# NUSTM/FacialMMT

Hardware: AMD Instinct MI355X
Metric: utterances/sec T+A+V forward+bwd, 160-frame face seq, 1/2/4/8 GPU (higher is better)
Workload: dtype bf16; 1 GPU; configs[1]: T+A+V, RoBERTa-large (random init), 160-frame face seq (uint8 112x112 crops, fused pil-bicubic x2 + normalise), batch 4 utterances/GPU, bf16, fwd+bwd+clip+AdamW every step; global_batch=4, parallelism=dp1, hip_graphs=whole step: 2 graphs (fwd+bwd | clip+optimizer), text_encoder_concurrent_with_swin=True, swin_forward_pipelined_across_steps=False, text_encoder_parameters=bf16 with fp32 master weights in the optimizer

## Files before the change

### facialmmt_amd/_lib.py

```python
from __future__ import annotations

import ctypes as C
import os

_HERE = os.path.dirname(os.path.abspath(__file__))
LIB_PATH = os.path.join(_HERE, "libfmmt_hip.so")

F32, BF16 = 0, 1
GENERIC = 0x100
EPI_NONE, EPI_GELU, EPI_GELU_BWD, EPI_GELU_DG, EPI_MUL_AUX = 0, 1, 2, 3, 4
SAVE_DG = 0x200
BATCH_MAJOR = 0x400
RESIZE_PIL, RESIZE_CV2 = 0, 1

_p, _i, _f, _sz, _u64 = C.c_void_p, C.c_int, C.c_float, C.c_size_t, C.c_uint64

SIGNATURES = {
    "fmmt_version": (_i, []),
    "fmmt_linear_fwd": (_i, [_i, _i, _i, _i, _p, _i, _p, _i, _p, _p, _i, _p, _i, _p, _i, _p, _i, _p, _i, _p]),
    "fmmt_linear_splitk_workspace": (_sz, [_i, _i, _i]),
    "fmmt_linear_fwd_splitk": (_i, [_i, _i, _i, _i, _p, _i, _p, _i, _p, _p, _i, _p, _sz, _p]),
    "fmmt_linear_wgrad_workspace": (_sz, [_i, _i, _i, _i]),
    "fmmt_linear_wgrad": (_i, [_i, _i, _i, _i, _p, _i, _p, _i, _p, _p, _p, _i, _i, _p, _sz, _p]),
    "fmmt_linear_wgrad_partials": (_i, [_i, _i, _i, _i, _p, _i, _p, _i, _i, _p, _i, _i, _p, _sz, _p]),
# ... 86 lines not shown
DIGEST_WORDS = 6

EVAL_SHARD_SIGNATURES = {
    "fmmt_eval_accumulate_rows": (_i, [_i, _i, _i, _p, _i, _p, _p, _p, _p, _p, _p, _p, _p, _p, C.c_int64, _p]),
    "fmmt_eval_merge": (_i, [_i, _i, C.c_int64, C.c_int64, _p, _p, _p, _p, _p, _p, _p]),
}

JITTER_SIGNATURES = {
    "fmmt_jitter_table_check": (_i, [_p, _i]),
    "fmmt_patch_embed_u8_jitter": (_i, [_i, _i, _i, _i, _p, _p, _p, _p, _p, _p, _p]),
    "fmmt_patch_embed_u8_jitter_ln_fwd": (_i, [_i, _i, _i, _i, _p, _p, _p, _p, _p, _p, _p, _p, _p, _f, _p, _p, _p, _p, _p, _p]),
}
JITTER_WORDS, JITTER_BANDS = 8, 56
JITTER_BRIGHTNESS, JITTER_CONTRAST, JITTER_SATURATION, JITTER_HUE, JITTER_NONE = 0, 1, 2, 3, 4

AUG_SIGNATURES = {
    "fmmt_aug_table_check": (_i, [_p, _i]),
    "fmmt_aug_workspace_bytes": (C.c_size_t, [_i]),
    "fmmt_patch_embed_u8_aug": (_i, [_i, _i, _i, _i, _p, _p, _p, _p, _p, _p, C.c_size_t, _p, _p]),
    "fmmt_patch_embed_u8_aug_ln_fwd": (_i, [_i, _i, _i, _i, _p, _p, _p, _p, _p, _p, C.c_size_t, _p, _p, _p, _p, _f, _p, _p, _p, _p, _p, _p]),
}
AUG_WORDS, AUG_FLAG_GRAY, AUG_MAX_RADIUS, AUG_HALO = 20, 1, 1, 6

FMMT_EINVAL, FMMT_EALIGN, FMMT_EWORKSPACE = -1, -2, -3
_ERR = {-1: "FMMT_EINVAL (bad shape / unsupported size)", -2: "FMMT_EALIGN (pointer or leading dimension not 16-byte aligned)",
        -3: "FMMT_EWORKSPACE (workspace too small)"}

_lib = None


class FmmtError(RuntimeError):
    pass


def load():
    global _lib
    if _lib is not None:
        return _lib
    if not os.path.exists(LIB_PATH):
        raise FmmtError(f"{LIB_PATH} is missing: build it with `python -m facialmmt_amd.build` "
                        f"(or __graft_entry__.build()); there is no CPU / PyTorch fallback for the hot path")
    lib = C.CDLL(LIB_PATH)
    for name, (res, args) in list(SIGNATURES.items()) + list(POOL_HEAD_SIGNATURES.items()) + list(RAGGED_SIGNATURES.items()) + list(EVAL_COLLECT_SIGNATURES.items()) + list(POOL_HEAD_ROWS_SIGNATURES.items()) + list(GUARD_SIGNATURES.items()) + list(DIGEST_SIGNATURES.items()) + list(EVAL_SHARD_SIGNATURES.items()) + list(JITTER_SIGNATURES.items()) + list(AUG_SIGNATURES.items()):
        fn = getattr(lib, name)
        fn.restype = res
        fn.argtypes = args
    _lib = lib
    return lib


def check(rc: int, what: str):
    if rc != 0:
        msg = _ERR.get(rc, f"hipError_t {rc}")
        raise FmmtError(f"{what} failed: {msg}")


def dtype_code(t) -> int:
    import torch
    if t == torch.float32:
        return F32
    if t == torch.bfloat16:
        return BF16
    raise FmmtError(f"unsupported activation dtype {t}: the HIP path computes in float32 (parity) or bfloat16 (throughput)")
```

### facialmmt_amd/build.py

```python
from __future__ import annotations

import glob
import os
import subprocess
import sys
from concurrent.futures import ThreadPoolExecutor

HERE = os.path.dirname(os.path.abspath(__file__))
CSRC = os.path.join(HERE, "csrc")
OUT = os.path.join(HERE, "libfmmt_hip.so")
SOURCES = ["gemm.hip", "layernorm.hip", "attn.hip", "wattn_mfma.hip", "wattn_bwd_ref.hip", "wblock.hip", "wblock_ref.hip", "mha_mfma.hip", "misc.hip", "preproc.hip", "mlp_fused.hip", "mlp_ref.hip", "patch_ln.hip", "lin_lnbwd.hip", "plm_fused.hip", "frame_filter.hip", "eval.hip", "pool_head.hip", "ragged.hip", "guard.hip", "digest.hip", "eval_shard.hip", "color_jitter.hip", "aff_augment.hip"]
FLAGS = ["--offload-arch=gfx950", "-O3", "-std=c++17", "-fPIC", "-ffp-contract=fast"]


def _stale(target, deps):
    if not os.path.exists(target):
        return True
    t = os.path.getmtime(target)
    return any(os.path.getmtime(d) > t for d in deps)


def build(force: bool = False, verbose: bool = True, tag: str = "") -> str:
    hipcc = os.environ.get("HIPCC", "/opt/rocm/bin/hipcc")
    tag = tag or os.environ.get("FMMT_BUILD_TAG", "")
    csrc = os.environ.get("FMMT_CSRC_DIR", CSRC) if tag else CSRC
    headers = sorted(glob.glob(os.path.join(csrc, "*.h"))) + [os.path.join(csrc, "..", "..", "include", h) for h in ("fmmt.h", "fmmt_pool_head.h", "fmmt_ragged.h", "fmmt_eval_collect.h", "fmmt_pool_head_rows.h", "fmmt_guard.h", "fmmt_digest.h", "fmmt_eval_shard.h", "fmmt_jitter.h", "fmmt_aug.h")]
    objdir = os.path.join(HERE, "build_" + tag if tag else "build")
    out = os.path.join(HERE, f"libfmmt_hip_{tag}.so") if tag else OUT
    os.makedirs(objdir, exist_ok=True)
    jobs = []
    for s in SOURCES:
        src = os.path.join(csrc, s)
        obj = os.path.join(objdir, s.replace(".hip", ".o"))
        if force or _stale(obj, [src] + headers):
            jobs.append((src, obj))

    def cc(job):
        src, obj = job
        cmd = [hipcc] + FLAGS + os.environ.get("FMMT_CFLAGS", "").split() + ["-c", src, "-o", obj]
        if verbose:
            print(" ".join(cmd), flush=True)
        subprocess.run(cmd, check=True)

    with ThreadPoolExecutor(max_workers=4) as ex:
        list(ex.map(cc, jobs))
    objs = [os.path.join(objdir, s.replace(".hip", ".o")) for s in SOURCES]
    if force or jobs or _stale(out, objs):
        cmd = [hipcc, "--offload-arch=gfx950", "-shared", "-fPIC", "-o", out] + objs
        if verbose:
# ... 8 lines not shown
```

### facialmmt_amd/csrc/gemm.hip

```cpp
#include "gemm_common.h"
#include "gemm_ph.h"
#include "gemm_ph3.h"
#include <stdlib.h>
#include <type_traits>

namespace {

template <typename T> struct Mma;
template <> struct Mma<bf16> {
    static constexpr int KM = 32;
    static constexpr int KP = 8;
    using frag = bf16x8;
    static __device__ __forceinline__ f32x4 mma(frag a, frag b, f32x4 c) {
        return __builtin_amdgcn_mfma_f32_16x16x32_bf16(a, b, c, 0, 0, 0);
    }
    static __device__ __forceinline__ frag load(const bf16* p) { return *reinterpret_cast<const bf16x8*>(p); }
};
template <> struct Mma<float> {
    static constexpr int KM = 4;
    static constexpr int KP = 1;
    using frag = float;
    static __device__ __forceinline__ f32x4 mma(frag a, frag b, f32x4 c) {
        return __builtin_amdgcn_mfma_f32_16x16x4f32(a, b, c, 0, 0, 0);
    }
    static __device__ __forceinline__ frag load(const float* p) { return *p; }
};

__device__ __forceinline__ int xcd_remap(int bid, int nwg) {
    const int q = nwg >> 3, r = nwg & 7, xcd = bid & 7;
    return (xcd < r ? xcd * (q + 1) : r * (q + 1) + (xcd - r) * q) + (bid >> 3);
}

template <int BM, int NBUF> struct NtWaves { static constexpr int value = (BM == 128) ? (NBUF == 1 ? 3 : 2) : 4; };
template <typename T, int BM, int BN, int BK, int NBUF, bool GLDS, bool SEG = false>
__global__ __launch_bounds__(256) __attribute__((amdgpu_waves_per_eu(NtWaves<BM, NBUF>::value)))
void linear_nt_kernel(LinArgs p) {
    constexpr int VEC = Vec<T>::N;
    static_assert(!SEG || GLDS, "segmented weights: direct-to-LDS kernels only");
    constexpr int PITCH = GLDS ? BK : BK + VEC;
    constexpr int KM = Mma<T>::KM, KP = Mma<T>::KP;
    constexpr int WM = BM / 2, WN = BN / 2, MT = WM / 16, NT = WN / 16;
    constexpr int KV = BK / VEC;
    constexpr int W_VECS = BN * KV, X_VECS = BM * KV;
    constexpr int WV = (W_VECS + 255) / 256, XV = (X_VECS + 255) / 256;
    constexpr int CW = 4 * NT;

    extern __shared__ __attribute__((aligned(16))) char smem[];
    T* Ws = reinterpret_cast<T*>(smem);
    T* Xs = Ws + NBUF * BN * PITCH;

    const int tid = threadIdx.x, lane = tid & 63, wave = tid >> 6;
    const int wm = wave >> 1, wn = wave & 1;
    const int li = lane & 15, lg = lane >> 4;

    const T* __restrict__ xg = reinterpret_cast<const T*>(p.x);
    const T* __restrict__ wg = reinterpret_cast<const T*>(p.w);
    const float* bias_seg = nullptr;
    if constexpr (SEG) {
        if (p.wseg_mode == 1) {
            const int s_ = ((xcd_remap(blockIdx.x, gridDim.x) % p.tiles_n) * BN) / p.wseg;
            wg = reinterpret_cast<const T*>(s_ == 0 ? p.w : (s_ == 1 ? p.w1 : p.w2)) - (ptrdiff_t)s_ * p.wseg * p.ldw;
            const float* bs_ = s_ == 0 ? p.bias : (s_ == 1 ? p.bias1 : p.bias2);
            bias_seg = bs_ ? bs_ - (ptrdiff_t)s_ * p.wseg : nullptr;
        }
    }

    const int kbeg = p.ksplit ? blockIdx.y * p.ksplit : 0;
    const int kend = p.ksplit ? min(p.K, kbeg + p.ksplit) : p.K;
    const int nk = (kend - kbeg + BK - 1) / BK;

    struct Stage { Vec<T> w[WV], x[XV]; };
    Stage R0;

    auto gload = [&](Stage& R, int k0, int m0, int n0) {
#pragma unroll
        for (int i = 0; i < WV; ++i) {
            const int v = tid + i * 256;
            if (v < W_VECS) {
                const int row = v / KV, kc = (v % KV) * VEC;
                const int n = min(n0 + row, p.N - 1);
                R.w[i] = (k0 + kc < kend) ? ldvec<T>(wg + (size_t)n * p.ldw + k0 + kc) : zerovec<T>();
            }
        }
#pragma unroll
        for (int i = 0; i < XV; ++i) {
            const int v = tid + i * 256;
            if (v < X_VECS) {
                const int row = v / KV, kc = (v % KV) * VEC;
                const int m = min(m0 + row, p.M - 1);
                R.x[i] = (k0 + kc < kend) ? ldvec<T>(xg + (size_t)m * p.ldx + k0 + kc) : zerovec<T>();
            }
        }
// ... 44 lines not shown
#pragma unroll
            for (int a = 0; a < MT; ++a)
#pragma unroll
                for (int b = 0; b < NT; ++b) acc[a][b] = Mma<T>::mma(wf[b], xf[a], acc[a][b]);
        }
    };

    auto epilogue = [&](int m0, int n0) {
        if constexpr (SEG) {
            if (bias_seg) {
#pragma unroll
                for (int b = 0; b < NT; ++b) {
                    const f32x4 bb = *reinterpret_cast<const f32x4*>(bias_seg + n0 + wn * WN + chan_of<CW>(b, lg, 0));
#pragma unroll
                    for (int a = 0; a < MT; ++a) acc[a][b] += bb;
                }
            }
            nt_epilogue<T, MT, NT, true>(p, acc, m0 + wm * WM, n0 + wn * WN, li, lg);
        } else {
            nt_epilogue<T, MT, NT>(p, acc, m0 + wm * WM, n0 + wn * WN, li, lg);
        }
    };

    const int logical = xcd_remap(blockIdx.x, gridDim.x);
    const int m0 = (logical / p.tiles_n) * BM, n0 = (logical % p.tiles_n) * BN;
#pragma unroll
    for (int a = 0; a < MT; ++a)
#pragma unroll
        for (int b = 0; b < NT; ++b) acc[a][b] = f32x4{0.f, 0.f, 0.f, 0.f};
    if constexpr (GLDS) {
        static_assert(BK == 64 && (NBUF == 2 || NBUF == 4) && sizeof(T) == 2, "direct-to-LDS path: bf16, BK = 64, two or four buffers");
        typedef __attribute__((address_space(1))) const void gptr_t;
        typedef __attribute__((address_space(3))) void lptr_t;
        auto issue = [&](int buf, int k0) {
            const int r8 = lane >> 3, c = lane & 7;
            const T* wk = wg;
            int kw = k0;
            if constexpr (SEG) {
                if (p.wseg_mode == 2) {
                    const int s_ = k0 / p.wseg;
                    wk = reinterpret_cast<const T*>(s_ == 0 ? p.w : (s_ == 1 ? p.w1 : p.w2));
                    kw = k0 - s_ * p.wseg;
                }
            }
#pragma unroll
            for (int i = 0; i < BN / 32; ++i) {
                const int grp = i * 4 + wave, row = grp * 8 + r8;
// ... 31 lines not shown
            const int cur = kt & 1;
            if (kt + 1 < nk) issue(cur ^ 1, kbeg + (kt + 1) * BK);
            compute(cur);
            __syncthreads();
        }
        epilogue(m0, n0);
        return;
    }
    gload(R0, kbeg, m0, n0);
    lstore(R0, 0);
    __syncthreads();
    if constexpr (NBUF == 1) {
        compute(0);
    } else {
        for (int kt = 0; kt < nk; ++kt) {
            const int cur = kt & 1;
            if (kt + 1 < nk) gload(R0, kbeg + (kt + 1) * BK, m0, n0);
            compute(cur);
            if (kt + 1 < nk) lstore(R0, cur ^ 1);
            __syncthreads();
        }
    }
    epilogue(m0, n0);
}

__global__ __launch_bounds__(512) void linear_nt_deep_kernel(LinArgs p) {
    using T = bf16;
    constexpr int BM = 256, BN = 128, BK = 64, PITCH = 64, MT = 4, NT = 4, CW = 16;
    constexpr int STAGE = (BM + BN) * PITCH;
    extern __shared__ __attribute__((aligned(16))) char smem[];
    T* S = reinterpret_cast<T*>(smem);

    const int tid = threadIdx.x, lane = tid & 63, wave = tid >> 6;
    const int wm = wave >> 1, wn = wave & 1;
    const int li = lane & 15, lg = lane >> 4;
    const int logical = xcd_remap(blockIdx.x, gridDim.x);
    const int m0 = (logical / p.tiles_n) * BM, n0 = (logical % p.tiles_n) * BN;
    const T* __restrict__ xg = reinterpret_cast<const T*>(p.x);
    const T* __restrict__ wg = reinterpret_cast<const T*>(p.w);
    const int nk = p.K / BK;

    typedef __attribute__((address_space(1))) const void gptr_t;
    typedef __attribute__((address_space(3))) void lptr_t;
    const int r8 = lane >> 3, c = lane & 7;
    auto issue = [&](int buf, int k0) {
        T* base = S + buf * STAGE;
// ... 677 lines not shown
    if (a.rowscale && a.rows_per_scale <= 0) return 0;
    if ((unsigned long long)a.M * a.ldx >= (1ull << 31) || (unsigned long long)a.N * a.ldw >= (1ull << 31) || (unsigned long long)a.M * a.ldy >= (1ull << 31) ||
        (a.res && (unsigned long long)a.M * a.ldres >= (1ull << 31)))
        return 0;
    if (a.N % 256) {
        if (gelu_pre || a.K > 512) return 0;
        const long long t384 = (long long)((a.M + 383) / 384) * (a.N / 128), r384 = (t384 + 255) / 256;
        if (t384 < 256 || t384 * 100 < r384 * 256 * 85) return 0;
        *epi3 = mul_aux ? 6 : has_op ? 5 : 2;
        return 4;
    }
    const long long t256 = (long long)((a.M + 255) / 256) * (a.N / 256), t192 = (long long)((a.M + 191) / 192) * (a.N / 256);
    const long long r256 = (t256 + 255) / 256, r192 = (t192 + 255) / 256;
    const long long min_tiles = a.M < 16384 ? 150 : 256;
    const bool ok256 = t256 >= min_tiles && (a.M < 16384 || t256 * 100 >= r256 * 256 * 85);
    const bool ok192 = t192 >= min_tiles && (a.M < 16384 || t192 * 100 >= r192 * 256 * 85);
    *epi3 = gelu_pre ? 3 : mul_aux ? 6 : has_op ? 5 : 2;
    if (gelu_pre || has_op || mul_aux) return ok192 ? 3 : 0;
    const long long c256 = r256 * 256 * 100, c192 = r192 * 192 * 103;
    if (ok192 && (!ok256 || c192 < c256)) return 3;
    return ok256 ? 1 : 0;
}

template <typename T>
int dispatch_nt(const LinArgs& a, hipStream_t st) {
    const bool n96 = (a.N % 96 == 0) && (a.N % 128 != 0);
    if (a.M <= 4096 && (a.N < 16384 || a.M < 256)) {
        if constexpr (sizeof(T) == 2) {
            constexpr int SMALL_TILES = 256;
            constexpr int SMALL_R4K = 2048;
            const int tiles = ((a.M + 63) / 64) * ((a.N + 127) / 128);
            if (tiles < SMALL_TILES && a.N % 64 == 0 && a.K % 64 == 0 && a.K >= 128 && !a.ksplit && a.ldx % 8 == 0 && a.ldw % 8 == 0) {
                if (a.K >= SMALL_R4K) return launch_nt<T, 32, 64, 64, 4, true>(a, st);
                return launch_nt<T, 32, 64, 64, 2, true>(a, st);
            }
        }
        return n96 ? dispatch_nt_bk<T, 64, 96>(a, st) : dispatch_nt_bk<T, 64, 128>(a, st);
    }
    if constexpr (sizeof(T) == 2) {
        int epi3 = 2;
        if (const int ph = ph_plan(a, &epi3)) {
            if (ph == 1) return launch_ph<2>(a, st);
            if (ph == 4) return epi3 == 6 ? launch_ph3<6, true, 4>(a, st) : epi3 == 5 ? launch_ph3<5, true, 4>(a, st) : launch_ph3<2, true, 4>(a, st);
            return epi3 == 3 ? launch_ph3<3>(a, st) : epi3 == 6 ? launch_ph3<6>(a, st) : epi3 == 5 ? launch_ph3<5>(a, st) : launch_ph3<2>(a, st);
        }
        if (const int bn = p256_plan(a))
            return bn == 256 ? launch_p256<256, 64, 2>(a, st) : bn == 192 ? launch_p256<192, 64, 2>(a, st) : launch_p256<128, 64, 3>(a, st);
        constexpr int DEEP_MINM = 65536, DEEP_MINK = 96;
        const bool big = a.M >= DEEP_MINM && !a.ksplit && a.K % 32 == 0 && a.K >= DEEP_MINK && a.ldx % 8 == 0 && a.ldw % 8 == 0 &&
                         !(a.K == 96 && a.epi == FMMT_EPI_GELU);
        if (big && (a.N % 128 == 0 || n96)) {
            constexpr size_t lds = (size_t)3 * (256 + 128) * 64 * 2;
            constexpr size_t lds96 = (size_t)3 * (256 + 96) * 32 * 2;
            static FmmtLdsOnce lds_once[7];
            {
                const void* fns[] = {reinterpret_cast<const void*>(&linear_nt_deep_kernel),
                                     reinterpret_cast<const void*>(&linear_nt_deep32_kernel<0, 128>),
                                     reinterpret_cast<const void*>(&linear_nt_deep32_kernel<6, 128>),
// ... 256 lines not shown
        for (int e = 0; e < VEC; ++e) bsum[rowgrp * 128 + cchunk * VEC + e] = colsum[e];
        __syncthreads();
        if (tid < 128) {
            float t = 0.f;
            for (int g = 0; g < 256 / CV; ++g) t += bsum[g * 128 + tid];
            if (n0 + tid < p.N) p.part_b[(size_t)split * p.N + n0 + tid] = t;
        }
    }
}

template <typename T, int BMS, bool FEW = false, int PF = 1>
int launch_tn(const TnArgs& a, dim3 grid, hipStream_t st) {
    constexpr int VEC = Vec<T>::N;
    constexpr size_t lds = (size_t)4 * BMS * (sizeof(T) == 2 ? 128 : 128 + VEC) * sizeof(T) + (256 / (128 / VEC)) * 128 * sizeof(float);
    static FmmtLdsOnce lds_once;
    if (lds > 65536) {
        if (int rc_ = lds_once.set(reinterpret_cast<const void*>(&linear_tn_kernel<T, BMS, FEW, PF>), (int)lds)) return rc_;
    }
    hipLaunchKernelGGL((linear_tn_kernel<T, BMS, FEW, PF>), grid, dim3(256), lds, st, a);
    FMMT_CHECK_LAUNCH();
    return 0;
}

__global__ __launch_bounds__(512) void linear_tn_few_kernel(TnArgs p) {
    using T = bf16;
    constexpr int WS = 2 * 32 * 64;
    extern __shared__ __attribute__((aligned(16))) char smem[];
    T* stage = reinterpret_cast<T*>(smem);
    const int tid = threadIdx.x, lane = tid & 63;
    const int wave = __builtin_amdgcn_readfirstlane(tid >> 6);
    const int li = lane & 15, lg = lane >> 4;
    const int tile_n = blockIdx.x / p.tiles_k, tile_k = blockIdx.x % p.tiles_k;
    const int n0 = tile_n * 64, k0 = tile_k * 64;
    if (p.hdr && blockIdx.x == 0 && tid == 0) { p.hdr[0] = 1; p.hdr[1] = 0; p.hdr[2] = p.N; }
    const T* __restrict__ dyg = reinterpret_cast<const T*>(p.dy);
    const T* __restrict__ xg = reinterpret_cast<const T*>(p.x);
    const bool do_bias = p.part_b != nullptr && tile_k == 0;
    const int mbeg = wave * p.chunk, mend = min(p.M, mbeg + p.chunk);
    const int nsteps = mend > mbeg ? (mend - mbeg + 31) / 32 : 0;
    T* my = stage + wave * WS;

    const int lr = lane >> 3, lc = lane & 7;
    auto f = [](int row) { return ((row >> 1) & 1) | (((row >> 3) & 1) << 1); };
    bf16x8 ra[4], rb[4];
    auto load = [&](int m0) {
#pragma unroll
        for (int i = 0; i < 4; ++i) {
            const int m = m0 + lr + 8 * i;
            if (m < mend) {
                ra[i] = *reinterpret_cast<const bf16x8*>(dyg + (size_t)m * p.lddy + n0 + lc * 8);
                rb[i] = *reinterpret_cast<const bf16x8*>(xg + (size_t)m * p.ldx + k0 + lc * 8);
            } else {
#pragma unroll
                for (int e = 0; e < 8; ++e) { ra[i][e] = (bf16)0.f; rb[i][e] = (bf16)0.f; }
            }
        }
    };
// ... 67 lines not shown
#pragma unroll
                for (int b = 0; b < 4; ++b) acc[a][b] += *reinterpret_cast<const f32x4*>(src + (a * 4 + b) * 256);
                accb[a] += *reinterpret_cast<const f32x4*>(src + (16 + a) * 256);
            }
        }
    }
    if (wave != 0) return;
#pragma unroll
    for (int a = 0; a < 4; ++a)
#pragma unroll
        for (int b = 0; b < 4; ++b) {
            const int k = k0 + b * 16 + li;
#pragma unroll
            for (int r = 0; r < 4; ++r) p.part_w[(size_t)(n0 + a * 16 + lg * 4 + r) * p.K + k] = acc[a][b][r];
        }
    if (do_bias && li == 0) {
#pragma unroll
        for (int a = 0; a < 4; ++a)
#pragma unroll
            for (int r = 0; r < 4; ++r) p.part_b[n0 + a * 16 + lg * 4 + r] = accb[a][r];
    }
}

int launch_tn_few(int M, int N, int K, const void* dy, int lddy, const void* x, int ldx, float* dw, float* db, int* hdr, hipStream_t st) {
    constexpr int lds = 80 * 1024;
    static FmmtLdsOnce lds_once;
    if (int rc_ = lds_once.set(reinterpret_cast<const void*>(&linear_tn_few_kernel), lds)) return rc_;
    TnArgs a{M, N, K, dy, lddy, x, ldx, dw, db, nullptr, 1, K / 64, (M + 7) / 8, N / 64, 0, hdr, 1};
    hipLaunchKernelGGL(linear_tn_few_kernel, dim3((N / 64) * (K / 64)), dim3(512), lds, st, a);
    FMMT_CHECK_LAUNCH();
    return 0;
}

bool tn_few_ok(int M, int N, int K, int dtype) {
    return dtype == FMMT_BF16 && M > 128 && M <= 2048 && N % 64 == 0 && K % 64 == 0 && (N / 64) * (K / 64) >= 8 && (N / 64) * (K / 64) <= 1024;
}

__device__ __forceinline__ int tn_swz2(int row) { return ((row >> 1) & 1) | (((row >> 3) & 1) << 1); }
template <int CH>
__device__ __forceinline__ int tn_sigma(int row, int blk) {
    if constexpr (CH == 192) return blk < 8 ? (blk ^ tn_swz(row)) : 8 + ((blk & 3) ^ tn_swz2(row));
    else return blk ^ tn_swz(row);
}


#define FMMT_TR2(o0, o1, ad, im) "ds_read_b64_tr_b16 %" #o0 ", %" #ad "\n\tds_read_b64_tr_b16 %" #o1 ", %" #ad " offset:%" #im "\n\t"
template <int FA, int OFFA, int OFFB>
__device__ __forceinline__ void tn_read12(s16x4 (&o)[24], const unsigned (&ad)[12]) {
    static_assert(FA == 8 || FA == 6, "fragment split");
    if constexpr (FA == 8) {
        asm volatile(FMMT_TR2(0, 1, 24, 36) FMMT_TR2(2, 3, 25, 36) FMMT_TR2(4, 5, 26, 36) FMMT_TR2(6, 7, 27, 36)
                     FMMT_TR2(8, 9, 28, 36) FMMT_TR2(10, 11, 29, 36) FMMT_TR2(12, 13, 30, 36) FMMT_TR2(14, 15, 31, 36)
                     FMMT_TR2(16, 17, 32, 37) FMMT_TR2(18, 19, 33, 37) FMMT_TR2(20, 21, 34, 37) FMMT_TR2(22, 23, 35, 37)
                     "s_waitcnt lgkmcnt(0)"
                     : "=&v"(o[0]), "=&v"(o[1]), "=&v"(o[2]), "=&v"(o[3]), "=&v"(o[4]), "=&v"(o[5]), "=&v"(o[6]), "=&v"(o[7]),
                       "=&v"(o[8]), "=&v"(o[9]), "=&v"(o[10]), "=&v"(o[11]), "=&v"(o[12]), "=&v"(o[13]), "=&v"(o[14]), "=&v"(o[15]),
                       "=&v"(o[16]), "=&v"(o[17]), "=&v"(o[18]), "=&v"(o[19]), "=&v"(o[20]), "=&v"(o[21]), "=&v"(o[22]), "=&v"(o[23])
                     : "v"(ad[0]), "v"(ad[1]), "v"(ad[2]), "v"(ad[3]), "v"(ad[4]), "v"(ad[5]), "v"(ad[6]), "v"(ad[7]),
// ... 609 lines not shown
    const int wblocks = (int)(((size_t)rows * K / 4 + 63) / 64), bblocks = db ? (rows / 4 + 63) / 64 : 0;
    hipLaunchKernelGGL(reduce_partials_kernel, dim3(wblocks + bblocks), dim3(64 * RP_GROUPS), 0, st, part_w, dw, nw, hdr, wblocks, part_b, db, (size_t)N, K);
    FMMT_CHECK_LAUNCH();
    return 0;
}

extern "C" int fmmt_linear_wgrad(int dtype, int M, int N, int K,
                                 const void* dy, int lddy, const void* x, int ldx,
                                 float* dw, float* db, const float* rowscale, int rows_per_scale, int x_epi,
                                 void* workspace, size_t workspace_bytes, void* stream) {
    if (!aligned16(dw)) return FMMT_EALIGN;
    const bool few = M > 0 && N > 0 && K > 0 && tn_few_ok(M, N, K, dtype) && !rowscale && !x_epi && lddy % 8 == 0 && ldx % 8 == 0;
    if (M > 0 && N > 0 && K > 0 && (dtype == FMMT_BF16 || dtype == FMMT_F32) && (few || tn_smax(M, N, K, dtype) == 1)) {
        const int vec = dtype == FMMT_BF16 ? 8 : 4;
        if (N % vec || K % vec || lddy % vec || ldx % vec) return FMMT_EINVAL;
        if (rowscale && rows_per_scale <= 0) return FMMT_EINVAL;
        if (!aligned16(dy) || !aligned16(x)) return FMMT_EALIGN;
        return launch_tn_plan(dtype, M, N, K, dy, lddy, x, ldx, dw, db, rowscale, rows_per_scale, x_epi, nullptr, reinterpret_cast<hipStream_t>(stream));
    }
    if (int rc = fmmt_linear_wgrad_partials(dtype, M, N, K, dy, lddy, x, ldx, db != nullptr, rowscale, rows_per_scale, x_epi,
                                            workspace, workspace_bytes, stream)) return rc;
    return fmmt_linear_wgrad_finish(dtype, M, N, K, dw, db, workspace, workspace_bytes, stream);
}
```

### facialmmt_amd/ops.py

```python
from __future__ import annotations

import math
import weakref

import torch
from torch.autograd import Function

from . import _lib
from ._lib import EPI_GELU, EPI_GELU_BWD, EPI_GELU_DG, EPI_MUL_AUX, EPI_NONE, SAVE_DG, check, dtype_code


def _st():
    return torch.cuda.current_stream().cuda_stream


def _p(t):
    return None if t is None else t.data_ptr()


def _c16(t: torch.Tensor) -> torch.Tensor:
    t = t.contiguous()
    return t.clone() if t.data_ptr() % 16 else t


# ... 40 lines not shown


def wgrad_raw(dy2, x2, want_bias, rowscale=None, rows_per_scale=1, x_gelu=False, out=None):
    M, N = dy2.shape
    K = x2.shape[1]
    lib = _lib.load()
    if out is not None:
        dw, db = out
        assert dw.shape == (N, K) and dw.dtype == torch.float32 and dw.is_contiguous() and (not want_bias or (db.shape == (N,) and db.is_contiguous()))
    else:
        dw = torch.empty((N, K), dtype=torch.float32, device=dy2.device)
        db = torch.empty((N,), dtype=torch.float32, device=dy2.device) if want_bias else None
    nbytes = lib.fmmt_linear_wgrad_workspace(dtype_code(dy2.dtype), M, N, K)
    ws = _ws(nbytes, dy2.device)
    if M <= 2048:
        rc = lib.fmmt_linear_wgrad(dtype_code(dy2.dtype), M, N, K, _p(dy2), N, _p(x2), K, _p(dw), _p(db), _p(rowscale), rows_per_scale,
                                   EPI_GELU if x_gelu else EPI_NONE, _p(ws), nbytes, _st())
        check(rc, f"fmmt_linear_wgrad(M={M},N={N},K={K})")
        return dw, db
    wgrad_partials_raw(dy2, x2, want_bias, ws, nbytes, rowscale, rows_per_scale, x_gelu)
    rc = lib.fmmt_linear_wgrad_finish(dtype_code(dy2.dtype), M, N, K, _p(dw), _p(db), _p(ws), nbytes, _st())
    check(rc, f"fmmt_linear_wgrad_finish(M={M},N={N},K={K})")
    return dw, db


_CAST_CACHE: dict = {}


def _lp(w: torch.Tensor, dtype, transpose: bool = False) -> torch.Tensor:
    base = w._base if w._base is not None else w
    wd = w.detach()
    if wd.dtype == dtype and not transpose:
        return wd.contiguous()
    capturing = wd.is_cuda and torch.cuda.is_current_stream_capturing()
    key = (w.storage_offset(), tuple(w.shape), tuple(w.stride()), dtype, transpose)
    if capturing and _PIN_SCOPE:
        pin = _PINNED.get(id(base))
        if pin is not None and key in pin:
            return pin[key]
    sub = None if capturing else _CAST_CACHE.get(id(base))
    if sub is not None:
        hit = sub.get(key)
        if hit is not None and hit[0] == w._version:
            return hit[1]
    out = wd.to(dtype)
    out = out.t().contiguous() if transpose else out.contiguous()
# ... 76 lines not shown
class LinearFn(Function):
    @staticmethod
    def forward(ctx, x, weight, bias, res, rowscale, rows_per_scale):
        _need_cuda(x, "linear")
        K = x.shape[-1]
        x2 = x.reshape(-1, K).contiguous()
        w = _lp(weight, x.dtype)
        res2 = res.reshape(-1, weight.shape[0]).contiguous() if res is not None else None
        y = linear_raw(x2, w, bias.detach() if bias is not None else None, res=res2, rowscale=rowscale,
                       rows_per_scale=rows_per_scale)
        ctx.save_for_backward(x2, weight, rowscale)
        ctx.has_bias = bias is not None
        ctx.has_res = res is not None
        ctx.rps = rows_per_scale
        ctx.xshape = x.shape
        return y.reshape(*x.shape[:-1], weight.shape[0])

    @staticmethod
    def backward(ctx, dy):
        x2, weight, rowscale = ctx.saved_tensors
        N = weight.shape[0]
        dy2 = dy.reshape(-1, N).contiguous()
        dx = dw = db = None
        if ctx.needs_input_grad[0]:
            dx = linear_raw(dy2, _lp(weight, dy2.dtype, transpose=True), None, rowscale=rowscale, rows_per_scale=ctx.rps).reshape(ctx.xshape)
        if ctx.needs_input_grad[1] or (ctx.has_bias and ctx.needs_input_grad[2]):
            dw, db = wgrad_raw(dy2, x2, ctx.has_bias, rowscale, ctx.rps)
        dres = dy if ctx.has_res else None
        return dx, dw, db, dres, None, None


def linear(x, weight, bias=None, res=None, rowscale=None, rows_per_scale=1):
    return LinearFn.apply(x, weight, bias, res, rowscale, rows_per_scale)


class InProjFn(Function):

    @staticmethod
    def forward(ctx, query, key, weight, bias):
        _need_cuda(query, "in_proj")
        E = weight.shape[1]
        q2 = query.reshape(-1, E).contiguous()
        k2 = key.reshape(-1, E).contiguous()
        wq, wkv = weight[:E], weight[E:]
        bq, bkv = (bias.detach()[:E], bias.detach()[E:]) if bias is not None else (None, None)
        q = linear_raw(q2, _lp(wq, query.dtype), bq)
        kv = linear_raw(k2, _lp(wkv, key.dtype), bkv)
        ctx.save_for_backward(q2, k2, weight)
        ctx.has_bias = bias is not None
        ctx.shapes = (query.shape, key.shape)
        return q.reshape(*query.shape[:-1], E), kv.reshape(*key.shape[:-1], 2 * E)

    @staticmethod
    def backward(ctx, dq, dkv):
        q2, k2, weight = ctx.saved_tensors
        E = weight.shape[1]
        dq2 = dq.reshape(-1, E).contiguous()
        dkv2 = dkv.reshape(-1, 2 * E).contiguous()
        dquery = dkey = dw = db = None
        if ctx.needs_input_grad[0]:
            dquery = linear_raw(dq2, _lp(weight[:E], dq2.dtype, transpose=True), None).reshape(ctx.shapes[0])
        if ctx.needs_input_grad[1]:
            dkey = linear_raw(dkv2, _lp(weight[E:], dkv2.dtype, transpose=True), None).reshape(ctx.shapes[1])
        if ctx.needs_input_grad[2] or (ctx.has_bias and ctx.needs_input_grad[3]):
            dw = torch.empty((3 * E, E), dtype=torch.float32, device=dq2.device)
            db = torch.empty((3 * E,), dtype=torch.float32, device=dq2.device) if ctx.has_bias else None
            wgrad_raw(dq2, q2, ctx.has_bias, out=(dw[:E], db[:E] if db is not None else None))
            wgrad_raw(dkv2, k2, ctx.has_bias, out=(dw[E:], db[E:] if db is not None else None))
        return dquery, dkey, dw, db


def in_proj_q_kv(query, key, weight, bias):
    return InProjFn.apply(query, key, weight, bias)


def colsum_raw(x2, out_dtype=None):
    M, N = x2.shape
    out_dtype = out_dtype or x2.dtype
    out = torch.empty((N,), dtype=out_dtype, device=x2.device)
    check(_lib.load().fmmt_colsum(dtype_code(x2.dtype), dtype_code(out_dtype), M, N, _p(x2), N, _p(out), _st()), f"fmmt_colsum(M={M},N={N})")
    return out


class PlmLayerNormFn(torch.autograd.Function):

    @staticmethod
    def forward(ctx, x, weight, bias, eps):
        ctx.save_for_backward(x, weight)
        ctx.eps = eps
        return torch.nn.functional.layer_norm(x, (x.shape[-1],), weight, bias, eps)

    @staticmethod
# ... 313 lines not shown
        x2 = x.reshape(-1, K).contiguous()
        w1l, w2l = _lp(w1, x.dtype), _lp(w2, x.dtype)
        train = grad_on and any(ctx.needs_input_grad)
        h_pre = torch.empty((x2.shape[0], w1.shape[0]), dtype=x.dtype, device=x.device) if train else None
        res2 = res.reshape(-1, w2.shape[0]).contiguous() if res is not None else None
        if _mlp_fusable(x2, w1, w2, b1, b2):
            h = torch.empty_like(h_pre) if (train and _MLP_SAVE_H) else None
            ctx.dg = mlp_saves_dg(x2, w1, w2, b1, b2)
            y = mlp_fused_raw(x2, w1l, b1.detach().float().contiguous(), w2l, b2.detach().float().contiguous(), res2, rowscale, rows_per_scale, h_pre, h, ctx.dg)
        else:
            ctx.dg = mlp_saves_dg(x2, w1, w2, b1, b2)
            h = linear_raw(x2, w1l, b1.detach(), epi=EPI_GELU_DG if ctx.dg else EPI_GELU, y_pre=h_pre)
            y = linear_raw(h, w2l, b2.detach(), res=res2, rowscale=rowscale, rows_per_scale=rows_per_scale)
        ctx.save_for_backward(x2, w1, w2, h_pre, h, rowscale)
        ctx.rps = rows_per_scale
        ctx.has_res = res is not None
        ctx.xshape = x.shape
        return y.reshape(*x.shape[:-1], w2.shape[0])

    @staticmethod
    def backward(ctx, dy):
        x2, w1, w2, h_pre, h, rowscale = ctx.saved_tensors
        dy2 = dy.reshape(-1, w2.shape[0]).contiguous()
        dh = linear_raw(dy2, _lp(w2, dy2.dtype, transpose=True), None, epi=EPI_MUL_AUX if ctx.dg else EPI_GELU_BWD, aux=h_pre, rowscale=rowscale,
                        rows_per_scale=ctx.rps)
        dw2, db2 = wgrad_raw(dy2, h, True, rowscale, ctx.rps) if h is not None else wgrad_raw(dy2, h_pre, True, rowscale, ctx.rps, x_gelu=True)
        dx = linear_raw(dh, _lp(w1, dy2.dtype, transpose=True), None).reshape(ctx.xshape) if ctx.needs_input_grad[0] else None
        dw1, db1 = wgrad_raw(dh, x2, True)
        return dx, dw1, db1, dw2, db2, (dy if ctx.has_res else None), None, None, None


_MLP_BWD_FUSED = True
_MLP_BWD_WIDTHS = (96, 192)
_MLP_BWD_LN = True


def mlp_bwd_input_raw(dy2, h_pre, w1, w2, rowscale, rows_per_scale, dg=False):
    M, C = dy2.shape
    dt = dy2.dtype
    if _MLP_BWD_FUSED and _mlp_dtype_ok(dt) and C in _MLP_BWD_WIDTHS and w1.shape == (4 * C, C) and M >= 4096:
        dh = torch.empty((M, 4 * C), dtype=dt, device=dy2.device)
        dx = torch.empty_like(dy2)
        w2t, w1t = _lp(w2, dt, transpose=True), _lp(w1, dt, transpose=True)
        rc = _lib.load().fmmt_mlp_bwd_input(dtype_code(dt) | (SAVE_DG if dg else 0), M, C, _p(dy2), _p(h_pre), _p(w2t), _p(w1t),
                                            _p(rowscale), rows_per_scale, _p(dh), _p(dx), _st())
        check(rc, f"fmmt_mlp_bwd_input(M={M},C={C})")
        return dh, dx
    dh = linear_raw(dy2, _lp(w2, dt, transpose=True), None, epi=EPI_MUL_AUX if dg else EPI_GELU_BWD, aux=h_pre, rowscale=rowscale, rows_per_scale=rows_per_scale)
    return dh, linear_raw(dh, _lp(w1, dt, transpose=True), None)


class MlpLnFn(Function):
# ... 1186 lines not shown
```

### include/fmmt.h

```cpp
#ifndef FMMT_H
#define FMMT_H
#include <stddef.h>
#include <stdint.h>

#ifdef __cplusplus
extern "C" {
#endif

#define FMMT_F32 0
#define FMMT_BF16 1
#define FMMT_GENERIC 0x100
#define FMMT_SAVE_DG 0x200
#define FMMT_BATCH_MAJOR 0x400

#define FMMT_EINVAL (-1)
#define FMMT_EALIGN (-2)
#define FMMT_EWORKSPACE (-3)

#define FMMT_EPI_GELU 1
#define FMMT_EPI_GELU_BWD 2
#define FMMT_EPI_GELU_DG 3
#define FMMT_EPI_MUL_AUX 4

int fmmt_version(void);
// ... 162 lines not shown
                        const float* lut_dev, void* cols, void* stream);

int fmmt_patch_embed_ln_fwd(int dtype, int M, int C, int K, const void* cols, const void* w, const float* bias, const float* ln_gamma,
                            const float* ln_beta, float eps, void* x_pre, void* y, float* mean, float* rstd, void* stream);

int fmmt_patch_embed_u8_ln_fwd(int dtype, int mode, int n_img, int in_size, const void* img_u8, const int32_t* table_dev, const float* lut_dev,
                               const void* w, const float* bias, const float* ln_gamma, const float* ln_beta, float eps,
                               void* cols, void* x_pre, void* y, float* mean, float* rstd, void* stream);

int fmmt_emotion_head_fwd(int dtype, int N, int K, int H, int NL, const void* feats, int ld, const float* w1, const float* b1, const float* w2,
                          const float* b2, const float* gumbel, float tau, float* preds, float* importance, void* stream);
int fmmt_eval_accumulate(int dtype, int B, int NL, const void* logits, int ld, const int64_t* labels, double* loss_sum, int64_t* count,
                         int64_t* confusion, int32_t* pred, float* logits_out, int64_t out_offset, int64_t out_capacity, void* stream);

#include "fmmt_pool_head.h"
#include "fmmt_ragged.h"
#include "fmmt_eval_collect.h"
#include "fmmt_pool_head_rows.h"
#include "fmmt_guard.h"
#include "fmmt_digest.h"
#include "fmmt_eval_shard.h"
#include "fmmt_jitter.h"
#include "fmmt_aug.h"

#ifdef __cplusplus
}
#endif
#endif
```

Before: 73.97 utterances/s.

## Fuse small-M linear backward dgrad and wgrad into one co-scheduled kernel launch

Adds a combined backward kernel for linears with few rows: the dgrad GEMM (two 256-thread NT tiles hosted per 512-thread workgroup) and the wgrad TN-few kernel run as different workgroups of a single launch. The aim is to fill the GPU better on small-M backward GEMMs and cut one launch per linear, since each GEMM alone leaves compute units idle. Linear, in-proj q/kv and MLP backward use it when a heuristic says the dgrad tile count is small. In exchange, the NT body is refactored to take a logical block id, idle hosted halves must spin through matching barriers, and LDS per workgroup grows.

```diff
diff --git a/facialmmt_amd/_lib.py b/facialmmt_amd/_lib.py
--- a/facialmmt_amd/_lib.py
+++ b/facialmmt_amd/_lib.py
@@ -132,6 +132,11 @@
 }
 AUG_WORDS, AUG_FLAG_GRAY, AUG_MAX_RADIUS, AUG_HALO = 20, 1, 1, 6
 
+FEW_BWD_SIGNATURES = {
+    "fmmt_linear_bwd_few": (_i, [_i, _i, _i, _i, _p, _i, _p, _i, _p, _i, _p, _i, _i, _p, _i, _p, _p, _p]),
+    "fmmt_linear_bwd_few_pays": (_i, [_i, _i, _i]),
+}
+
 FMMT_EINVAL, FMMT_EALIGN, FMMT_EWORKSPACE = -1, -2, -3
 _ERR = {-1: "FMMT_EINVAL (bad shape / unsupported size)", -2: "FMMT_EALIGN (pointer or leading dimension not 16-byte aligned)",
         -3: "FMMT_EWORKSPACE (workspace too small)"}
@@ -151,7 +156,7 @@
         raise FmmtError(f"{LIB_PATH} is missing: build it with `python -m facialmmt_amd.build` "
                         f"(or __graft_entry__.build()); there is no CPU / PyTorch fallback for the hot path")
     lib = C.CDLL(LIB_PATH)
-    for name, (res, args) in list(SIGNATURES.items()) + list(POOL_HEAD_SIGNATURES.items()) + list(RAGGED_SIGNATURES.items()) + list(EVAL_COLLECT_SIGNATURES.items()) + list(POOL_HEAD_ROWS_SIGNATURES.items()) + list(GUARD_SIGNATURES.items()) + list(DIGEST_SIGNATURES.items()) + list(EVAL_SHARD_SIGNATURES.items()) + list(JITTER_SIGNATURES.items()) + list(AUG_SIGNATURES.items()):
+    for name, (res, args) in list(SIGNATURES.items()) + list(POOL_HEAD_SIGNATURES.items()) + list(RAGGED_SIGNATURES.items()) + list(EVAL_COLLECT_SIGNATURES.items()) + list(POOL_HEAD_ROWS_SIGNATURES.items()) + list(GUARD_SIGNATURES.items()) + list(DIGEST_SIGNATURES.items()) + list(EVAL_SHARD_SIGNATURES.items()) + list(JITTER_SIGNATURES.items()) + list(AUG_SIGNATURES.items()) + list(FEW_BWD_SIGNATURES.items()):
         fn = getattr(lib, name)
         fn.restype = res
         fn.argtypes = args
diff --git a/facialmmt_amd/build.py b/facialmmt_amd/build.py
--- a/facialmmt_amd/build.py
+++ b/facialmmt_amd/build.py
@@ -24,7 +24,7 @@
     hipcc = os.environ.get("HIPCC", "/opt/rocm/bin/hipcc")
     tag = tag or os.environ.get("FMMT_BUILD_TAG", "")
     csrc = os.environ.get("FMMT_CSRC_DIR", CSRC) if tag else CSRC
-    headers = sorted(glob.glob(os.path.join(csrc, "*.h"))) + [os.path.join(csrc, "..", "..", "include", h) for h in ("fmmt.h", "fmmt_pool_head.h", "fmmt_ragged.h", "fmmt_eval_collect.h", "fmmt_pool_head_rows.h", "fmmt_guard.h", "fmmt_digest.h", "fmmt_eval_shard.h", "fmmt_jitter.h", "fmmt_aug.h")]
+    headers = sorted(glob.glob(os.path.join(csrc, "*.h"))) + [os.path.join(csrc, "..", "..", "include", h) for h in ("fmmt.h", "fmmt_pool_head.h", "fmmt_ragged.h", "fmmt_eval_collect.h", "fmmt_pool_head_rows.h", "fmmt_guard.h", "fmmt_digest.h", "fmmt_eval_shard.h", "fmmt_jitter.h", "fmmt_aug.h", "fmmt_few_bwd.h")]
     objdir = os.path.join(HERE, "build_" + tag if tag else "build")
     out = os.path.join(HERE, f"libfmmt_hip_{tag}.so") if tag else OUT
     os.makedirs(objdir, exist_ok=True)
diff --git a/facialmmt_amd/csrc/gemm.hip b/facialmmt_amd/csrc/gemm.hip
--- a/facialmmt_amd/csrc/gemm.hip
+++ b/facialmmt_amd/csrc/gemm.hip
@@ -32,11 +32,11 @@
 }
 
 template <int BM, int NBUF> struct NtWaves { static constexpr int value = (BM == 128) ? (NBUF == 1 ? 3 : 2) : 4; };
-template <typename T, int BM, int BN, int BK, int NBUF, bool GLDS, bool SEG = false>
-__global__ __launch_bounds__(256) __attribute__((amdgpu_waves_per_eu(NtWaves<BM, NBUF>::value)))
-void linear_nt_kernel(LinArgs p) {
+template <typename T, int BM, int BN, int BK, int NBUF, bool GLDS, bool SEG = false, bool HOSTED = false>
+__device__ __forceinline__ void linear_nt_body(const LinArgs& p, char* smem, const int bid, const int nblk) {
     constexpr int VEC = Vec<T>::N;
     static_assert(!SEG || GLDS, "segmented weights: direct-to-LDS kernels only");
+    static_assert(!HOSTED || (GLDS && !SEG), "hosted in a 512-thread workgroup: the direct-to-LDS kernels only");
     constexpr int PITCH = GLDS ? BK : BK + VEC;
     constexpr int KM = Mma<T>::KM, KP = Mma<T>::KP;
     constexpr int WM = BM / 2, WN = BN / 2, MT = WM / 16, NT = WN / 16;
@@ -45,11 +45,10 @@
     constexpr int WV = (W_VECS + 255) / 256, XV = (X_VECS + 255) / 256;
     constexpr int CW = 4 * NT;
 
-    extern __shared__ __attribute__((aligned(16))) char smem[];
     T* Ws = reinterpret_cast<T*>(smem);
     T* Xs = Ws + NBUF * BN * PITCH;
 
-    const int tid = threadIdx.x, lane = tid & 63, wave = tid >> 6;
+    const int tid = HOSTED ? (threadIdx.x & 255) : threadIdx.x, lane = tid & 63, wave = tid >> 6;
     const int wm = wave >> 1, wn = wave & 1;
     const int li = lane & 15, lg = lane >> 4;
 
@@ -58,7 +57,7 @@
     const float* bias_seg = nullptr;
     if constexpr (SEG) {
         if (p.wseg_mode == 1) {
-            const int s_ = ((xcd_remap(blockIdx.x, gridDim.x) % p.tiles_n) * BN) / p.wseg;
+            const int s_ = ((xcd_remap(bid, nblk) % p.tiles_n) * BN) / p.wseg;
             wg = reinterpret_cast<const T*>(s_ == 0 ? p.w : (s_ == 1 ? p.w1 : p.w2)) - (ptrdiff_t)s_ * p.wseg * p.ldw;
             const float* bs_ = s_ == 0 ? p.bias : (s_ == 1 ? p.bias1 : p.bias2);
             bias_seg = bs_ ? bs_ - (ptrdiff_t)s_ * p.wseg : nullptr;
@@ -68,6 +67,18 @@
     const int kbeg = p.ksplit ? blockIdx.y * p.ksplit : 0;
     const int kend = p.ksplit ? min(p.K, kbeg + p.ksplit) : p.K;
     const int nk = (kend - kbeg + BK - 1) / BK;
+
+    if constexpr (HOSTED) {
+        if (bid >= nblk) {
+            if constexpr (NBUF == 4) {
+                for (int kt = 0; kt < nk; ++kt) __builtin_amdgcn_s_barrier();
+            } else {
+                __syncthreads();
+                for (int kt = 0; kt < nk; ++kt) __syncthreads();
+            }
+            return;
+        }
+    }
 
     struct Stage { Vec<T> w[WV], x[XV]; };
     Stage R0;
@@ -158,7 +169,7 @@
         }
     };
 
-    const int logical = xcd_remap(blockIdx.x, gridDim.x);
+    const int logical = xcd_remap(bid, nblk);
     const int m0 = (logical / p.tiles_n) * BM, n0 = (logical % p.tiles_n) * BN;
 #pragma unroll
     for (int a = 0; a < MT; ++a)
@@ -236,6 +247,13 @@
         }
     }
     epilogue(m0, n0);
+}
+
+template <typename T, int BM, int BN, int BK, int NBUF, bool GLDS, bool SEG = false>
+__global__ __launch_bounds__(256) __attribute__((amdgpu_waves_per_eu(NtWaves<BM, NBUF>::value)))
+void linear_nt_kernel(LinArgs p) {
+    extern __shared__ __attribute__((aligned(16))) char smem[];
+    linear_nt_body<T, BM, BN, BK, NBUF, GLDS, SEG>(p, smem, blockIdx.x, gridDim.x);
 }
 
 __global__ __launch_bounds__(512) void linear_nt_deep_kernel(LinArgs p) {
@@ -959,18 +977,24 @@
     return ok256 ? 1 : 0;
 }
 
+int nt_few_plan(const LinArgs& a) {
+    if (!(a.M <= 4096 && (a.N < 16384 || a.M < 256)) || a.ksplit || a.K % 64 || a.ldx % 8 || a.ldw % 8) return 0;
+    constexpr int SMALL_TILES = 256;
+    constexpr int SMALL_R4K = 2048;
+    const int tiles = ((a.M + 63) / 64) * ((a.N + 127) / 128);
+    if (tiles < SMALL_TILES && a.N % 64 == 0 && a.K >= 128) return a.K >= SMALL_R4K ? 2 : 1;
+    if ((a.N % 96 == 0 && a.N % 128 != 0) || a.K <= 64 || (a.K >= 2048 && tiles <= 256)) return 0;
+    return 3;
+}
+
 template <typename T>
 int dispatch_nt(const LinArgs& a, hipStream_t st) {
     const bool n96 = (a.N % 96 == 0) && (a.N % 128 != 0);
     if (a.M <= 4096 && (a.N < 16384 || a.M < 256)) {
         if constexpr (sizeof(T) == 2) {
-            constexpr int SMALL_TILES = 256;
-            constexpr int SMALL_R4K = 2048;
-            const int tiles = ((a.M + 63) / 64) * ((a.N + 127) / 128);
-            if (tiles < SMALL_TILES && a.N % 64 == 0 && a.K % 64 == 0 && a.K >= 128 && !a.ksplit && a.ldx % 8 == 0 && a.ldw % 8 == 0) {
-                if (a.K >= SMALL_R4K) return launch_nt<T, 32, 64, 64, 4, true>(a, st);
-                return launch_nt<T, 32, 64, 64, 2, true>(a, st);
-            }
+            const int few = nt_few_plan(a);
+            if (few == 2) return launch_nt<T, 32, 64, 64, 4, true>(a, st);
+            if (few == 1) return launch_nt<T, 32, 64, 64, 2, true>(a, st);
         }
         return n96 ? dispatch_nt_bk<T, 64, 96>(a, st) : dispatch_nt_bk<T, 64, 128>(a, st);
     }
@@ -1273,17 +1297,16 @@
     return 0;
 }
 
-__global__ __launch_bounds__(512) void linear_tn_few_kernel(TnArgs p) {
+__device__ __forceinline__ void linear_tn_few_body(const TnArgs& p, char* smem, const int bid) {
     using T = bf16;
     constexpr int WS = 2 * 32 * 64;
-    extern __shared__ __attribute__((aligned(16))) char smem[];
     T* stage = reinterpret_cast<T*>(smem);
     const int tid = threadIdx.x, lane = tid & 63;
     const int wave = __builtin_amdgcn_readfirstlane(tid >> 6);
     const int li = lane & 15, lg = lane >> 4;
-    const int tile_n = blockIdx.x / p.tiles_k, tile_k = blockIdx.x % p.tiles_k;
+    const int tile_n = bid / p.tiles_k, tile_k = bid % p.tiles_k;
     const int n0 = tile_n * 64, k0 = tile_k * 64;
-    if (p.hdr && blockIdx.x == 0 && tid == 0) { p.hdr[0] = 1; p.hdr[1] = 0; p.hdr[2] = p.N; }
+    if (p.hdr && bid == 0 && tid == 0) { p.hdr[0] = 1; p.hdr[1] = 0; p.hdr[2] = p.N; }
     const T* __restrict__ dyg = reinterpret_cast<const T*>(p.dy);
     const T* __restrict__ xg = reinterpret_cast<const T*>(p.x);
     const bool do_bias = p.part_b != nullptr && tile_k == 0;
@@ -1397,6 +1420,11 @@
     }
 }
 
+__global__ __launch_bounds__(512) void linear_tn_few_kernel(TnArgs p) {
+    extern __shared__ __attribute__((aligned(16))) char smem[];
+    linear_tn_few_body(p, smem, blockIdx.x);
+}
+
 int launch_tn_few(int M, int N, int K, const void* dy, int lddy, const void* x, int ldx, float* dw, float* db, int* hdr, hipStream_t st) {
     constexpr int lds = 80 * 1024;
     static FmmtLdsOnce lds_once;
@@ -1409,6 +1437,49 @@
 
 bool tn_few_ok(int M, int N, int K, int dtype) {
     return dtype == FMMT_BF16 && M > 128 && M <= 2048 && N % 64 == 0 && K % 64 == 0 && (N / 64) * (K / 64) >= 8 && (N / 64) * (K / 64) <= 1024;
+}
+
+struct BwdFewArgs {
+    LinArgs nt;
+    TnArgs tn;
+    int n_dx;
+};
+
+template <int BM, int BN, int NBUF>
+__global__ __launch_bounds__(512) void linear_bwd_few_kernel(BwdFewArgs p) {
+    constexpr int NT_LDS = NBUF * (BM + BN) * 64 * (int)sizeof(bf16);
+    extern __shared__ __attribute__((aligned(16))) char smem[];
+    const int bid = blockIdx.x, n_nt = (p.n_dx + 1) >> 1;
+    if (bid < n_nt) {
+        const int half = __builtin_amdgcn_readfirstlane(threadIdx.x >> 8);
+        linear_nt_body<bf16, BM, BN, 64, NBUF, true, false, true>(p.nt, smem + half * NT_LDS, 2 * bid + half, p.n_dx);
+    } else {
+        linear_tn_few_body(p.tn, smem, bid - n_nt);
+    }
+}
+
+int bwd_few_nt_workgroups(int M, int N, int K) {
+    if (!tn_few_ok(M, N, K, FMMT_BF16)) return 0;
+    LinArgs nt{M, K, N, nullptr, N, nullptr, N, nullptr, nullptr, K, nullptr, 0, nullptr, 0, nullptr, 0, nullptr, 1, 0, 0, 0, 0, nullptr};
+    const int plan = nt_few_plan(nt);
+    if (!plan) return 0;
+    const int bm = plan == 3 ? 64 : 32, bn = plan == 3 ? 128 : 64;
+    return (((M + bm - 1) / bm) * ((K + bn - 1) / bn) + 1) / 2;
+}
+
+template <int BM, int BN, int NBUF>
+int launch_bwd_few(const LinArgs& nt, const TnArgs& tn, hipStream_t st) {
+    constexpr int nt_lds = 2 * NBUF * (BM + BN) * 64 * (int)sizeof(bf16);
+    constexpr int lds = nt_lds > 80 * 1024 ? nt_lds : 80 * 1024;
+    static FmmtLdsOnce lds_once;
+    if (int rc_ = lds_once.set(reinterpret_cast<const void*>(&linear_bwd_few_kernel<BM, BN, NBUF>), lds)) return rc_;
+    BwdFewArgs p{nt, tn, 0};
+    p.nt.tiles_n = (nt.N + BN - 1) / BN;
+    p.nt.tiles_m = (nt.M + BM - 1) / BM;
+    p.n_dx = p.nt.tiles_m * p.nt.tiles_n;
+    hipLaunchKernelGGL((linear_bwd_few_kernel<BM, BN, NBUF>), dim3((p.n_dx + 1) / 2 + tn.tiles_n * tn.tiles_k), dim3(512), lds, st, p);
+    FMMT_CHECK_LAUNCH();
+    return 0;
 }
 
 __device__ __forceinline__ int tn_swz2(int row) { return ((row >> 1) & 1) | (((row >> 3) & 1) << 1); }
@@ -2064,3 +2135,29 @@
                                             workspace, workspace_bytes, stream)) return rc;
     return fmmt_linear_wgrad_finish(dtype, M, N, K, dw, db, workspace, workspace_bytes, stream);
 }
+
+extern "C" int fmmt_linear_bwd_few(int dtype, int M, int N, int K, const void* dy, int lddy, const void* x, int ldx, const void* wt, int ldwt,
+                                   void* dx, int lddx, int epi, const void* aux, int ldaux, float* dw, float* db, void* stream) {
+    if (dtype != FMMT_BF16 || M <= 0 || N <= 0 || K <= 0) return FMMT_EINVAL;
+    if (!dy || !x || !wt || !dx || !dw) return FMMT_EINVAL;
+    if (N % 8 || K % 8 || lddy % 8 || ldx % 8 || ldwt % 8 || lddx % 4) return FMMT_EINVAL;
+    if (lddy < N || ldx < K || ldwt < N || lddx < K) return FMMT_EINVAL;
+    if (epi != 0 && epi != FMMT_EPI_GELU_BWD && epi != FMMT_EPI_MUL_AUX) return FMMT_EINVAL;
+    if (epi != 0 && (!aux || ldaux % 4 || ldaux < K)) return FMMT_EINVAL;
+    if (!aligned16(dy) || !aligned16(x) || !aligned16(wt) || !aligned16(dx) || !aligned16(dw) || (epi != 0 && !aligned16(aux))) return FMMT_EALIGN;
+    if (!tn_few_ok(M, N, K, dtype)) return FMMT_EINVAL;
+    LinArgs nt{M, K, N, dy, lddy, wt, ldwt, nullptr, dx, lddx, nullptr, epi, epi ? aux : nullptr, ldaux, nullptr, 0, nullptr, 1, 0, 0, 0, 0, nullptr};
+    const int plan = nt_few_plan(nt);
+    if (!plan) return FMMT_EINVAL;
+    TnArgs tn{M, N, K, dy, lddy, x, ldx, dw, db, nullptr, 1, K / 64, (M + 7) / 8, N / 64, 0, nullptr, 1};
+    hipStream_t st = reinterpret_cast<hipStream_t>(stream);
+    if (plan == 1) return launch_bwd_few<32, 64, 2>(nt, tn, st);
+    if (plan == 2) return launch_bwd_few<32, 64, 4>(nt, tn, st);
+    return launch_bwd_few<64, 128, 2>(nt, tn, st);
+}
+
+extern "C" int fmmt_linear_bwd_few_pays(int M, int N, int K) {
+    if (M <= 0 || N <= 0 || K <= 0) return 0;
+    const int n_nt = bwd_few_nt_workgroups(M, N, K);
+    return n_nt > 0 && n_nt <= 128;
+}
diff --git a/facialmmt_amd/ops.py b/facialmmt_amd/ops.py
--- a/facialmmt_amd/ops.py
+++ b/facialmmt_amd/ops.py
@@ -86,6 +86,31 @@
     rc = lib.fmmt_linear_wgrad_finish(dtype_code(dy2.dtype), M, N, K, _p(dw), _p(db), _p(ws), nbytes, _st())
     check(rc, f"fmmt_linear_wgrad_finish(M={M},N={N},K={K})")
     return dw, db
+
+
+_LINEAR_BWD_PAIRED = True
+
+
+def linear_bwd_few_raw(dy2, x2, wt, want_bias, out=None, epi=EPI_NONE, aux=None, always=False):
+    M, N = dy2.shape
+    K = x2.shape[1]
+    if not _LINEAR_BWD_PAIRED or dy2.dtype != torch.bfloat16 or x2.dtype != dy2.dtype or wt.dtype != dy2.dtype or not 128 < M <= 2048:
+        return None
+    if not always and not _lib.load().fmmt_linear_bwd_few_pays(M, N, K):
+        return None
+    if out is not None:
+        dw, db = out
+        assert dw.shape == (N, K) and dw.dtype == torch.float32 and dw.is_contiguous() and (not want_bias or (db.shape == (N,) and db.is_contiguous()))
+    else:
+        dw = torch.empty((N, K), dtype=torch.float32, device=dy2.device)
+        db = torch.empty((N,), dtype=torch.float32, device=dy2.device) if want_bias else None
+    dx = torch.empty((M, K), dtype=dy2.dtype, device=dy2.device)
+    rc = _lib.load().fmmt_linear_bwd_few(dtype_code(dy2.dtype), M, N, K, _p(dy2), N, _p(x2), K, _p(wt), N, _p(dx), K, epi, _p(aux), K,
+                                         _p(dw), _p(db) if want_bias else None, _st())
+    if rc == _lib.FMMT_EINVAL:
+        return None
+    check(rc, f"fmmt_linear_bwd_few(M={M},N={N},K={K})")
+    return dx, dw, db
 
 
 _CAST_CACHE: dict = {}
@@ -208,11 +233,17 @@
         N = weight.shape[0]
         dy2 = dy.reshape(-1, N).contiguous()
         dx = dw = db = None
-        if ctx.needs_input_grad[0]:
-            dx = linear_raw(dy2, _lp(weight, dy2.dtype, transpose=True), None, rowscale=rowscale, rows_per_scale=ctx.rps).reshape(ctx.xshape)
-        if ctx.needs_input_grad[1] or (ctx.has_bias and ctx.needs_input_grad[2]):
+        want_w = ctx.needs_input_grad[1] or (ctx.has_bias and ctx.needs_input_grad[2])
+        dres = dy if ctx.has_res else None
+        wt = _lp(weight, dy2.dtype, transpose=True) if ctx.needs_input_grad[0] else None
+        if wt is not None and want_w and rowscale is None:
+            got = linear_bwd_few_raw(dy2, x2, wt, ctx.has_bias)
+            if got is not None:
+                return got[0].reshape(ctx.xshape), got[1], got[2], dres, None, None
+        if wt is not None:
+            dx = linear_raw(dy2, wt, None, rowscale=rowscale, rows_per_scale=ctx.rps).reshape(ctx.xshape)
+        if want_w:
             dw, db = wgrad_raw(dy2, x2, ctx.has_bias, rowscale, ctx.rps)
-        dres = dy if ctx.has_res else None
         return dx, dw, db, dres, None, None
 
 
@@ -243,17 +274,22 @@
         E = weight.shape[1]
         dq2 = dq.reshape(-1, E).contiguous()
         dkv2 = dkv.reshape(-1, 2 * E).contiguous()
-        dquery = dkey = dw = db = None
-        if ctx.needs_input_grad[0]:
-            dquery = linear_raw(dq2, _lp(weight[:E], dq2.dtype, transpose=True), None).reshape(ctx.shapes[0])
-        if ctx.needs_input_grad[1]:
-            dkey = linear_raw(dkv2, _lp(weight[E:], dkv2.dtype, transpose=True), None).reshape(ctx.shapes[1])
+        dw = db = None
         if ctx.needs_input_grad[2] or (ctx.has_bias and ctx.needs_input_grad[3]):
             dw = torch.empty((3 * E, E), dtype=torch.float32, device=dq2.device)
             db = torch.empty((3 * E,), dtype=torch.float32, device=dq2.device) if ctx.has_bias else None
-            wgrad_raw(dq2, q2, ctx.has_bias, out=(dw[:E], db[:E] if db is not None else None))
-            wgrad_raw(dkv2, k2, ctx.has_bias, out=(dw[E:], db[E:] if db is not None else None))
-        return dquery, dkey, dw, db
+        dins = []
+        for need, d2, in2, rows, shape in ((ctx.needs_input_grad[0], dq2, q2, slice(0, E), ctx.shapes[0]),
+                                           (ctx.needs_input_grad[1], dkv2, k2, slice(E, 3 * E), ctx.shapes[1])):
+            out = (dw[rows], db[rows] if db is not None else None) if dw is not None else None
+            wt = _lp(weight[rows], d2.dtype, transpose=True) if need else None
+            got = linear_bwd_few_raw(d2, in2, wt, ctx.has_bias, out=out) if (need and out is not None) else None
+            if got is None:
+                got = (linear_raw(d2, wt, None) if need else None,)
+                if out is not None:
+                    wgrad_raw(d2, in2, ctx.has_bias, out=out)
+            dins.append(got[0].reshape(shape) if need else None)
+        return dins[0], dins[1], dw, db
 
 
 def in_proj_q_kv(query, key, weight, bias):
@@ -613,12 +649,21 @@
     def backward(ctx, dy):
         x2, w1, w2, h_pre, h, rowscale = ctx.saved_tensors
         dy2 = dy.reshape(-1, w2.shape[0]).contiguous()
-        dh = linear_raw(dy2, _lp(w2, dy2.dtype, transpose=True), None, epi=EPI_MUL_AUX if ctx.dg else EPI_GELU_BWD, aux=h_pre, rowscale=rowscale,
-                        rows_per_scale=ctx.rps)
-        dw2, db2 = wgrad_raw(dy2, h, True, rowscale, ctx.rps) if h is not None else wgrad_raw(dy2, h_pre, True, rowscale, ctx.rps, x_gelu=True)
-        dx = linear_raw(dh, _lp(w1, dy2.dtype, transpose=True), None).reshape(ctx.xshape) if ctx.needs_input_grad[0] else None
-        dw1, db1 = wgrad_raw(dh, x2, True)
-        return dx, dw1, db1, dw2, db2, (dy if ctx.has_res else None), None, None, None
+        w2t, epi = _lp(w2, dy2.dtype, transpose=True), EPI_MUL_AUX if ctx.dg else EPI_GELU_BWD
+        got = linear_bwd_few_raw(dy2, h, w2t, True, epi=epi, aux=h_pre) if (h is not None and rowscale is None) else None
+        if got is not None:
+            dh, dw2, db2 = got
+        else:
+            dh = linear_raw(dy2, w2t, None, epi=epi, aux=h_pre, rowscale=rowscale, rows_per_scale=ctx.rps)
+            dw2, db2 = wgrad_raw(dy2, h, True, rowscale, ctx.rps) if h is not None else wgrad_raw(dy2, h_pre, True, rowscale, ctx.rps, x_gelu=True)
+        w1t = _lp(w1, dy2.dtype, transpose=True) if ctx.needs_input_grad[0] else None
+        got = linear_bwd_few_raw(dh, x2, w1t, True) if w1t is not None else None
+        if got is not None:
+            dx, dw1, db1 = got
+        else:
+            dx = linear_raw(dh, w1t, None) if w1t is not None else None
+            dw1, db1 = wgrad_raw(dh, x2, True)
+        return (dx.reshape(ctx.xshape) if dx is not None else None), dw1, db1, dw2, db2, (dy if ctx.has_res else None), None, None, None
 
 
 _MLP_BWD_FUSED = True
diff --git a/include/fmmt.h b/include/fmmt.h
--- a/include/fmmt.h
+++ b/include/fmmt.h
@@ -208,6 +208,7 @@
 #include "fmmt_eval_shard.h"
 #include "fmmt_jitter.h"
 #include "fmmt_aug.h"
+#include "fmmt_few_bwd.h"
 
 #ifdef __cplusplus
 }
diff --git a/include/fmmt_few_bwd.h b/include/fmmt_few_bwd.h
--- /dev/null
+++ b/include/fmmt_few_bwd.h
@@ -0,0 +1,18 @@
+#ifndef FMMT_FEW_BWD_H
+#define FMMT_FEW_BWD_H
+#include <stddef.h>
+#include <stdint.h>
+
+#ifdef __cplusplus
+extern "C" {
+#endif
+
+int fmmt_linear_bwd_few(int dtype, int M, int N, int K, const void* dy, int lddy, const void* x, int ldx, const void* wt, int ldwt,
+                        void* dx, int lddx, int epi, const void* aux, int ldaux, float* dw, float* db, void* stream);
+
+int fmmt_linear_bwd_few_pays(int M, int N, int K);
+
+#ifdef __cplusplus
+}
+#endif
+#endif
```

Measured after the change: 74.04 utterances/s (median of 2 runs). No clear change (+0.1%).
